# MIT-SPARK/Khronos

Hardware: AMD Instinct MI355X
Metric: active-window frames/sec (+ Mvoxel-updates/sec) at 1280x720 RGB-D+labels, 2 cm voxels (higher is better)
Workload: dtype f32

## Files before the change

### khronos_amd/csrc/khr_kernels_fusion.h

```cpp
#pragma once
#include "khr_device.h"

namespace khr {


constexpr int kTile = 16;
constexpr int kMaxTick = 8;

__device__ inline void ingestTile(const float* __restrict__ depth_in, const uint8_t* __restrict__ rgb_in,
                                  const int32_t* __restrict__ label_in, float* __restrict__ depth, float* __restrict__ range,
                                  uint32_t* __restrict__ rgba, int32_t* __restrict__ label, int32_t* __restrict__ dyn,
                                  float* __restrict__ tile_max, int tile, int tw, int W, int H, float fx, float fy, float cx,
                                  float cy, int range_mode, float* d_out, float* r_out) {
  const int tx = tile % tw, ty = tile / tw;
  const int u = tx * kTile + (threadIdx.x & 15), v = ty * kTile + (threadIdx.x >> 4);
  float r = 0.f, d = 0.f;
  if (u < W && v < H) {
    const int i = v * W + u;
    d = depth_in[i];
    if (d > 0.f && isfinite(d)) {
      if (range_mode == 0) {
        r = d;
      } else {
        const float x = (static_cast<float>(u) - cx) / fx, y = (static_cast<float>(v) - cy) / fy;
// ... 208 lines not shown
struct TickFrusta {
  float R[kMaxTick][9], t[kMaxTick][3], max_range[kMaxTick];
  DevFrustum fr[kMaxTick];
};
constexpr int kTickAllocThreads = 1024;
__global__ __launch_bounds__(kTickAllocThreads) void k_tick_alloc(DevMap m, DevParams p, TickFrusta tf, int ncam, int3 lo, int3 dim,
                                                   uint32_t* __restrict__ work, uint32_t list_stride,
                                                   uint32_t* __restrict__ new_list, uint32_t* __restrict__ tick_counts, int epoch) {
  const int total = dim.x * dim.y * dim.z;
  const int i = blockIdx.x * blockDim.x + threadIdx.x;
  uint32_t seen = 0u;
  int bx = 0, by = 0, bz = 0;
  if (i < total) {
    bx = lo.x + i % dim.x;
    by = lo.y + (i / dim.x) % dim.y;
    bz = lo.z + i / (dim.x * dim.y);
    if (ownerOf(bx, by, bz, p.world) == p.rank) {
      for (int k = 0; k < ncam; ++k) {
        const DevFrustum& fr = tf.fr[k];
        if (abs(bx - fr.bc.x) > fr.n_steps || abs(by - fr.bc.y) > fr.n_steps || abs(bz - fr.bc.z) > fr.n_steps) continue;
        const bool in = blockIsCandidate(p, fr, tf.R[k], tf.t[k], tf.max_range[k], bx, by, bz);
        if (in) seen |= 1u << k;
      }
    }
  }
  const bool visible = seen != 0u;
  uint32_t slot = kInvalidSlot;
  const uint64_t key = packKey(bx, by, bz);
  if (visible) slot = htLookup(m, key);
  const bool need = visible && slot == kInvalidSlot;
  const uint32_t fidx = waveAggInc(&m.counters[C_FREE_HEAD], need);
  bool got = false;
  if (need) {
    if (fidx < m.counters[C_N_FREE]) {
      slot = m.free_slots[fidx];
      got = true;
      m.blk_index[slot] = make_int4(bx, by, bz, epoch);
      m.blk_flags[slot] = BLK_LIVE | BLK_TRACK_DIRTY | BLK_ANY_KEEP;
      m.mesh_desc[slot] = MeshDesc{0u, 0u};
      htInsertUnique(m, key, slot);
      atomicMax(&m.counters[C_MAX_SLOT], slot + 1);
    } else {
      atomicAdd(&m.counters[C_POOL_EXHAUSTED], 1u);
      slot = kInvalidSlot;
    }
  }
  const uint32_t nidx = waveAggInc(&m.counters[C_N_NEW], got);
  if (got) new_list[nidx] = slot;
  if (slot == kInvalidSlot) seen = 0u;
  __shared__ uint32_t s_cnt[kMaxTick], s_base[kMaxTick];
  if (threadIdx.x < kMaxTick) s_cnt[threadIdx.x] = 0u;
  __syncthreads();
  uint32_t loff[kMaxTick];
#pragma unroll
  for (int k = 0; k < kMaxTick; ++k) {
    loff[k] = 0u;
    if (k < ncam) loff[k] = waveAggInc(&s_cnt[k], ((seen >> k) & 1u) != 0u);
  }
  __syncthreads();
  if (threadIdx.x < static_cast<uint32_t>(ncam)) {
    const uint32_t n = s_cnt[threadIdx.x];
    s_base[threadIdx.x] = n ? atomicAdd(&tick_counts[2 * threadIdx.x], n) : 0u;
  }
  if (threadIdx.x == 64) {
    uint32_t tot = 0u;
    for (int k = 0; k < ncam; ++k) tot += s_cnt[k];
    if (tot) atomicAdd(&m.counters[C_N_VISIBLE], tot);
  }
  __syncthreads();
#pragma unroll
  for (int k = 0; k < kMaxTick; ++k)
    if (k < ncam && ((seen >> k) & 1u)) work[static_cast<size_t>(k) * list_stride + s_base[k] + loff[k]] = slot;
}

__global__ void k_begin_integrate(DevMap m, int nvox, uint32_t* wg_stats) {
  if (blockIdx.x == 0) beginIntegrate(m, nvox, wg_stats);
}
__global__ void k_tick_begin(DevMap m, int nvox, uint32_t* wg_stats, uint32_t* tick_counts, uint32_t extra_calls) {
  beginIntegrate(m, nvox, wg_stats);
  if (threadIdx.x < 6 * kMaxTick) tick_counts[threadIdx.x] = 0u;
  if (threadIdx.x == 0) m.stats[S_CUM_CALLS] += extra_calls;
}

__device__ inline void cullBlocks(const DevMap& m, const DevParams& p, const DevFrame& f, const uint32_t* __restrict__ work,
                                  const uint32_t* __restrict__ n_work, FuseList out, uint32_t wpb,
                                  uint32_t* __restrict__ n_tsdf, const float* __restrict__ tile_max, int tw, int th,
                                  uint32_t bid, uint32_t nblk, uint32_t* __restrict__ item_mask = nullptr, uint32_t cam = 0u) {
  constexpr int kPerWg = 8;
  __shared__ uint4 s_blk[kPerWg];
  __shared__ uint16_t s_item[4][kPerWg * kBandSlots];
  __shared__ uint32_t s_nkeep, s_ccnt[4], s_off[4];
  const uint32_t n = *n_work;
  const uint32_t lane = threadIdx.x & 63;
  for (uint32_t base = bid * kPerWg; base < n; base += nblk * kPerWg) {
  if (threadIdx.x == 0) s_nkeep = 0;
  if (threadIdx.x < 4) s_ccnt[threadIdx.x] = 0;
  __syncthreads();
  for (uint32_t wi = base + (threadIdx.x >> 6); wi < min(n, base + kPerWg); wi += 4) {
    const uint32_t slot = work[wi];
    const int4 bi = m.blk_index[slot];
    bool keep = true;
    if (tile_max) {
      const float margin = 1e-3f;
      const float lo[3] = {static_cast<float>(bi.x) * p.bs + 0.5f * p.vs, static_cast<float>(bi.y) * p.bs + 0.5f * p.vs,
                           static_cast<float>(bi.z) * p.bs + 0.5f * p.vs};
      const float ext = p.bs - p.vs;
      float zmin = 1e30f, zmax = -1e30f, umin = 1e30f, umax = -1e30f, vmin = 1e30f, vmax = -1e30f;
      float pcs[8][3];
#pragma unroll
      for (int k = 0; k < 8; ++k) {
        xform(f.R, f.t, lo[0] + ((k & 1) ? ext : 0.f), lo[1] + ((k & 2) ? ext : 0.f), lo[2] + ((k & 4) ? ext : 0.f), pcs[k]);
        zmin = fminf(zmin, pcs[k][2]);
        zmax = fmaxf(zmax, pcs[k][2]);
      }
      if (zmax <= -margin) keep = false;
      if (zmin > f.max_range + margin) keep = false;
      if (p.range_mode == 0 && zmax < f.min_range - margin) keep = false;
      if (keep && zmin > 0.05f) {
#pragma unroll
        for (int k = 0; k < 8; ++k) {
          const float u = (pcs[k][0] * f.fx) / pcs[k][2] + f.cx, v = (pcs[k][1] * f.fy) / pcs[k][2] + f.cy;
          umin = fminf(umin, u); umax = fmaxf(umax, u);
          vmin = fminf(vmin, v); vmax = fmaxf(vmax, v);
        }
        if (umax < -1.f || vmax < -1.f || umin > static_cast<float>(f.W) || vmin > static_cast<float>(f.H)) {
          keep = false;
        } else {
          const int tx0 = max(0, (static_cast<int>(floorf(umin)) - 1) / kTile);
          const int ty0 = max(0, (static_cast<int>(floorf(vmin)) - 1) / kTile);
          const int tx1 = min(tw - 1, (static_cast<int>(ceilf(umax)) + 2) / kTile);
          const int ty1 = min(th - 1, (static_cast<int>(ceilf(vmax)) + 2) / kTile);
          if (tx1 >= tx0 && ty1 >= ty0) {
            const int nx = tx1 - tx0 + 1, nt = nx * (ty1 - ty0 + 1);
            float mr = 0.f;
            for (int t = lane; t < nt; t += 64) mr = fmaxf(mr, tile_max[(ty0 + t / nx) * tw + tx0 + t % nx]);
#pragma unroll
            for (int o = 32; o > 0; o >>= 1) mr = fmaxf(mr, __shfl_xor(mr, o));
            if (mr < zmin - p.trunc - margin) keep = false;
          }
        }
      }
    }
    if (keep) {
      uint32_t kslot = 0;
      if (lane == 0) {
        kslot = atomicAdd(&s_nkeep, 1u);
        s_blk[kslot] = make_uint4(slot, static_cast<uint32_t>(bi.x), static_cast<uint32_t>(bi.y), static_cast<uint32_t>(bi.z));
      }
      kslot = __shfl(kslot, 0);
      const uint32_t lpi = 64u / wpb, item = lane / lpi, sub = lane % lpi;
      bool ikeep = true;
      if (tile_max && (p.dbg & 256) == 0) {
        const float margin = 1e-3f;
        const int patches = (p.vps * p.vps) >> 6, rows = 64 / p.vps, zr = p.vps / (static_cast<int>(wpb) / patches);
        const int y0 = (static_cast<int>(item) % patches) * rows, z0 = (static_cast<int>(item) / patches) * zr;
        const float lo[3] = {static_cast<float>(bi.x) * p.bs + 0.5f * p.vs, static_cast<float>(bi.y) * p.bs + (static_cast<float>(y0) + 0.5f) * p.vs,
                             static_cast<float>(bi.z) * p.bs + (static_cast<float>(z0) + 0.5f) * p.vs};
        const float ex[3] = {p.bs - p.vs, static_cast<float>(rows - 1) * p.vs, static_cast<float>(zr - 1) * p.vs};
        float zmin = 1e30f, zmax = -1e30f, umin = 1e30f, umax = -1e30f, vmin = 1e30f, vmax = -1e30f;
        float pcs[8][3];
#pragma unroll
        for (int k = 0; k < 8; ++k) {
          xform(f.R, f.t, lo[0] + ((k & 1) ? ex[0] : 0.f), lo[1] + ((k & 2) ? ex[1] : 0.f), lo[2] + ((k & 4) ? ex[2] : 0.f), pcs[k]);
          zmin = fminf(zmin, pcs[k][2]);
          zmax = fmaxf(zmax, pcs[k][2]);
        }
        if (zmax <= -margin) ikeep = false;
        if (zmin > f.max_range + margin) ikeep = false;
        if (p.range_mode == 0 && zmax < f.min_range - margin) ikeep = false;
        if (ikeep && zmin > 0.05f) {
#pragma unroll
          for (int k = 0; k < 8; ++k) {
            const float iz = __builtin_amdgcn_rcpf(pcs[k][2]);
            const float u = (pcs[k][0] * f.fx) * iz + f.cx, v = (pcs[k][1] * f.fy) * iz + f.cy;
            umin = fminf(umin, u); umax = fmaxf(umax, u);
            vmin = fminf(vmin, v); vmax = fmaxf(vmax, v);
          }
          if (umax < -2.f || vmax < -2.f || umin > static_cast<float>(f.W) + 1.f || vmin > static_cast<float>(f.H) + 1.f) {
            ikeep = false;
          } else {
            const int tx0 = max(0, (static_cast<int>(floorf(umin)) - 2) / kTile);
            const int ty0 = max(0, (static_cast<int>(floorf(vmin)) - 2) / kTile);
            const int tx1 = min(tw - 1, (static_cast<int>(ceilf(umax)) + 3) / kTile);
            const int ty1 = min(th - 1, (static_cast<int>(ceilf(vmax)) + 3) / kTile);
            const int nx = tx1 - tx0 + 1, nt = nx * (ty1 - ty0 + 1);
            if (tx1 >= tx0 && ty1 >= ty0 && nt <= 16 * static_cast<int>(lpi)) {
              float m0 = 0.f, m1 = 0.f;
              int t = static_cast<int>(sub);
              for (; t + static_cast<int>(lpi) < nt; t += 2 * static_cast<int>(lpi)) {
                const int t2 = t + static_cast<int>(lpi);
                const float a = tile_max[(ty0 + t / nx) * tw + tx0 + t % nx];
                const float b = tile_max[(ty0 + t2 / nx) * tw + tx0 + t2 % nx];
                m0 = fmaxf(m0, a);
                m1 = fmaxf(m1, b);
              }
              if (t < nt) m0 = fmaxf(m0, tile_max[(ty0 + t / nx) * tw + tx0 + t % nx]);
              float mr = fmaxf(m0, m1);
              for (uint32_t o = 1; o < lpi; o <<= 1) mr = fmaxf(mr, __shfl_xor(mr, static_cast<int>(o)));
              if (mr < zmin - p.trunc - margin) ikeep = false;
            }
          }
        }
      }
      if (ikeep && sub == 0 && item_mask) {
        const size_t mi = static_cast<size_t>(slot) * wpb + item;
        const uint32_t sh = 8u * static_cast<uint32_t>(mi & 3);
        const uint32_t old = atomicOr(&item_mask[mi >> 2], (1u << cam) << sh);
        if ((old >> sh) & 0xffu) ikeep = false;
      }
      if (ikeep && sub == 0) {
        const uint32_t cls = fuseClass(m.blk_band[static_cast<size_t>(slot) * kBandSlots + item] & kItemBandMask);
        s_item[cls][atomicAdd(&s_ccnt[cls], 1u)] = static_cast<uint16_t>((kslot << 8) | item);
      }
    }
  }
  __syncthreads();
  if (threadIdx.x < 4) s_off[threadIdx.x] = s_ccnt[threadIdx.x] ? atomicAdd(&out.counts[threadIdx.x], s_ccnt[threadIdx.x]) : 0u;
  if (threadIdx.x == 0 && s_nkeep) atomicAdd(n_tsdf, s_nkeep);
  __syncthreads();
#pragma unroll
  for (uint32_t cls = 0; cls < 4; ++cls) {
    for (uint32_t i = threadIdx.x; i < s_ccnt[cls]; i += blockDim.x) {
      const uint32_t it = s_item[cls][i];
      uint4 d = s_blk[it >> 8];
      d.x |= (it & 0xffu) << 24;
      *fuseDescPtr(out, cls, s_off[cls] + i) = d;
    }
  }
  __syncthreads();
  }
}

__global__ __launch_bounds__(256) void k_cull_blocks(DevMap m, DevParams p, DevFrame f,
                                                    const uint32_t* __restrict__ work, FuseList out, uint32_t wpb,
                                                    const float* __restrict__ tile_max, int tw, int th) {
  cullBlocks(m, p, f, work, &m.counters[C_N_VISIBLE], out, wpb, &m.counters[C_N_TSDF], tile_max, tw, th, blockIdx.x, gridDim.x);
}

struct TickFrames {
  DevFrame f[kMaxTick];
  const float* tile_max[kMaxTick];
};
__global__ __launch_bounds__(256) void k_tick_cull(DevMap m, DevParams p, TickFrames t, const uint32_t* __restrict__ work,
                                                  uint32_t list_stride, uint4* __restrict__ desc, uint32_t desc_stride, uint32_t wpb,
                                                  uint32_t* __restrict__ tick_counts, int use_tiles, int tw, int th,
                                                  uint32_t* __restrict__ item_mask) {
  const int cam = blockIdx.y;
  const int lc = item_mask ? 0 : cam;
  FuseList out{desc + static_cast<size_t>(2 * lc) * desc_stride, desc + static_cast<size_t>(2 * lc + 1) * desc_stride, desc_stride,
               &tick_counts[2 * kMaxTick + 4 * lc]};
  cullBlocks(m, p, t.f[cam], work + static_cast<size_t>(cam) * list_stride, &tick_counts[2 * cam], out, wpb, &tick_counts[2 * cam + 1],
             use_tiles ? t.tile_max[cam] : nullptr, tw, th, blockIdx.x, gridDim.x, item_mask, static_cast<uint32_t>(cam));
}

__global__ __launch_bounds__(256) void k_alloc_list(DevMap m, const int* __restrict__ idx, int n,
                                                   uint32_t* __restrict__ new_list) {
  const int i = blockIdx.x * blockDim.x + threadIdx.x;
  bool need = false;
  int bx = 0, by = 0, bz = 0;
  if (i < n) {
    bx = idx[3 * i];
    by = idx[3 * i + 1];
    bz = idx[3 * i + 2];
    need = htLookup(m, packKey(bx, by, bz)) == kInvalidSlot;
  }
  const uint32_t fidx = waveAggInc(&m.counters[C_FREE_HEAD], need);
  bool got = false;
  uint32_t slot = kInvalidSlot;
  if (need) {
    if (fidx < m.counters[C_N_FREE]) {
      slot = m.free_slots[fidx];
      got = true;
      m.blk_index[slot] = make_int4(bx, by, bz, 0);
      m.blk_flags[slot] = BLK_LIVE | BLK_TRACK_DIRTY | BLK_ANY_KEEP;
      m.mesh_desc[slot] = MeshDesc{0u, 0u};
      htInsertUnique(m, packKey(bx, by, bz), slot);
      atomicMax(&m.counters[C_MAX_SLOT], slot + 1);
    } else {
      atomicAdd(&m.counters[C_POOL_EXHAUSTED], 1u);
    }
  }
  const uint32_t nidx = waveAggInc(&m.counters[C_N_NEW], got);
  if (got) new_list[nidx] = slot;
}

__global__ __launch_bounds__(256) void k_list_live(DevMap m, uint32_t* __restrict__ work, uint32_t* counter,
                                                  uint32_t require_flags, FuseList out = FuseList{nullptr, nullptr, 0u, nullptr},
                                                  uint32_t wpb = 0u) {
  const uint32_t s = blockIdx.x * blockDim.x + threadIdx.x;
  bool live = false;
  if (s < m.counters[C_MAX_SLOT]) {
    const uint32_t fl = m.blk_flags[s];
    live = (fl & BLK_LIVE) && ((fl & require_flags) == require_flags);
  }
  const uint32_t idx = waveAggInc(counter, live);
  if (live) work[idx] = s;
  if (out.a) {
    const unsigned long long mask = __ballot(live);
    if (mask) {
      const uint32_t lane = laneId();
      const int leader = __ffsll(static_cast<long long>(mask)) - 1;
      uint32_t base = 0;
      if (lane == static_cast<uint32_t>(leader)) base = atomicAdd(&out.counts[3], static_cast<uint32_t>(__popcll(mask)) * wpb);
      base = __shfl(base, leader) + static_cast<uint32_t>(__popcll(mask & ((1ull << lane) - 1ull))) * wpb;
      if (live) {
        const int4 bi = m.blk_index[s];
        for (uint32_t it = 0; it < wpb; ++it)
          *fuseDescPtr(out, 3u, base + it) =
              make_uint4(s | (it << 24), static_cast<uint32_t>(bi.x), static_cast<uint32_t>(bi.y), static_cast<uint32_t>(bi.z));
      }
    }
  }
}

__device__ inline void initBlocks(const DevMap& m, const DevParams& p, const uint32_t* __restrict__ new_list, uint32_t bid,
                                  uint32_t nblk) {
  const uint32_t n = m.counters[C_N_NEW];
  const int nv = p.nvox;
  for (uint32_t b = bid; b < n; b += nblk) {
    const size_t slot = new_list[b];
    const uint4 z = make_uint4(0, 0, 0, 0);
    uint4* d4 = reinterpret_cast<uint4*>(m.dist + slot * nv);
    uint4* w4 = reinterpret_cast<uint4*>(m.weight + slot * nv);
    uint4* c4 = reinterpret_cast<uint4*>(m.color + slot * nv);
    uint4* l4 = reinterpret_cast<uint4*>(m.sem_label + slot * nv);
    for (int i = threadIdx.x; i < nv / 4; i += blockDim.x) {
      d4[i] = z;
      w4[i] = z;
      c4[i] = z;
      if (p.with_semantics) l4[i] = z;
    }
    uint4* f4 = reinterpret_cast<uint4*>(m.vflags + slot * nv);
    for (int i = threadIdx.x; i < nv / 16; i += blockDim.x) f4[i] = z;
    if (threadIdx.x < kBandSlots) m.blk_band[slot * kBandSlots + threadIdx.x] = 0;
    if (p.with_tracking) {
      uint4* o4 = reinterpret_cast<uint4*>(m.last_obs + slot * nv);
      uint4* q4 = reinterpret_cast<uint4*>(m.last_occ + slot * nv);
      for (int i = threadIdx.x; i < nv / 2; i += blockDim.x) {
        o4[i] = z;
        q4[i] = z;
      }
      uint64_t* fb = m.freebits + slot * (nv / 64);
      for (int i = threadIdx.x; i < nv / 64; i += blockDim.x) {
        fb[i] = 0ull;
        m.obs[slot * (nv / 64) + i] = make_ulonglong2(0ull, 0ull);
      }
    }
  }
}

__global__ __launch_bounds__(256) void k_init_blocks(DevMap m, DevParams p, const uint32_t* __restrict__ new_list) {
  initBlocks(m, p, new_list, blockIdx.x, gridDim.x);
}

__global__ __launch_bounds__(256) void k_init_cull(DevMap m, DevParams p, DevFrame f, const uint32_t* __restrict__ new_list,
                                                  const uint32_t* __restrict__ work, FuseList out, uint32_t wpb,
                                                  const float* __restrict__ tile_max, int tw, int th, uint32_t n_cull) {
  if (blockIdx.x < n_cull)
    cullBlocks(m, p, f, work, &m.counters[C_N_VISIBLE], out, wpb, &m.counters[C_N_TSDF], tile_max, tw, th, blockIdx.x, n_cull);
  else
    initBlocks(m, p, new_list, blockIdx.x - n_cull, gridDim.x - n_cull);
}

__device__ inline uint32_t foldItemRecords(uint32_t* __restrict__ blk_flags, uint16_t* __restrict__ blk_band, uint32_t s) {
  static_assert(kBandSlots == 32, "record row = 4 x 16 bytes");
  uint4* const row = reinterpret_cast<uint4*>(blk_band + static_cast<size_t>(s) * kBandSlots);
  uint32_t any = 0u;
  uint4 r[4];
#pragma unroll
  for (int i = 0; i < 4; ++i) {
    r[i] = row[i];
    any |= r[i].x | r[i].y | r[i].z | r[i].w;
  }
  const uint32_t tm = static_cast<uint32_t>(kItemTouched) * 0x00010001u, nm = static_cast<uint32_t>(kItemNeg) * 0x00010001u;
  uint32_t fl = blk_flags[s];
  if ((any & tm) == 0u) return fl;
  fl |= BLK_UPDATED | BLK_MESH_UPDATED | BLK_TRACKING_UPDATED | ((any & nm) ? BLK_HAS_NEG : 0u);
  blk_flags[s] = fl;
  const uint32_t keep = static_cast<uint32_t>(kItemBandMask) * 0x00010001u;
#pragma unroll
  for (int i = 0; i < 4; ++i) row[i] = make_uint4(r[i].x & keep, r[i].y & keep, r[i].z & keep, r[i].w & keep);
  return fl;
}
__global__ __launch_bounds__(256) void k_tracking_select(DevMap m, uint64_t lim_active, uint64_t lim_free, int force_full,
                                                        uint32_t* __restrict__ proc, uint32_t* __restrict__ ef_list,
                                                        uint32_t* __restrict__ cnt ,
                                                        uint32_t* __restrict__ cnt_next, uint16_t* __restrict__ fold_band) {
  const uint32_t s = blockIdx.x * blockDim.x + threadIdx.x;
  if (s == 0) { cnt_next[0] = 0u; cnt_next[1] = 0u; }
  bool need = false, touched = false, reload = false;
  if (s < m.counters[C_MAX_SLOT]) {
    const uint32_t fl = fold_band ? foldItemRecords(m.blk_flags, fold_band, s) : m.blk_flags[s];
    if (fl & BLK_LIVE) {
      touched = fl & BLK_TRACKING_UPDATED;
      need = force_full || (fl & (BLK_TRACKING_UPDATED | BLK_TRACK_DIRTY));
      reload = need;
      if (!need) {
        const ulonglong2 lim = reinterpret_cast<const ulonglong2*>(m.trk_lim)[s];
        need = !(lim_active <= lim.x && lim_free <= lim.y);
      }
    }
  }
  const uint32_t ip = waveAggInc(&cnt[0], need);
  if (need) {
    proc[ip] = s | (reload ? 0x80000000u : 0u);
    reinterpret_cast<ulonglong2*>(m.trk_lim)[s] = make_ulonglong2(~0ull, ~0ull);
    m.blk_flags[s] = m.blk_flags[s] & ~(BLK_TRACKING_UPDATED | BLK_HAS_ACTIVE | BLK_TRACK_DIRTY | BLK_ANY_KEEP);
  }
  const uint32_t ie = waveAggInc(&cnt[1], touched);
  if (touched) ef_list[ie] = s;
}

template <int VPS, int CH>
__global__ __launch_bounds__(256) void k_tracking_update(DevMap m, DevParams p, uint64_t stamp, uint64_t prev_stamp,
                                                        uint64_t lim_active, uint64_t lim_free,
                                                        const uint32_t* __restrict__ proc, const uint32_t* __restrict__ n_proc) {
  constexpr int NV = VPS * VPS * VPS;
  __shared__ uint64_t s_min[2][4];
  __shared__ uint32_t s_bits;
  const uint32_t n = *n_proc * CH;
  for (uint32_t wi = blockIdx.x; wi < n; wi += gridDim.x) {
    const uint32_t pe = proc[wi / CH];
    const uint32_t s = pe & 0x7fffffffu;
    const bool reload = (pe >> 31) != 0u;
    const int g0 = static_cast<int>(wi % CH) * (NV / 4 / CH);
    const size_t slot = s;
    const float4* __restrict__ dist4 = reinterpret_cast<const float4*>(m.dist + slot * NV);
    const ulonglong2* __restrict__ lobs2 = reinterpret_cast<const ulonglong2*>(m.last_obs + slot * NV);
    uint64_t* __restrict__ locc = m.last_occ + slot * NV;
    uint32_t* __restrict__ vfl4 = reinterpret_cast<uint32_t*>(m.vflags + slot * NV);
    uint64_t* __restrict__ fb = m.freebits + slot * (NV / 64);
    bool any_active = false, any_keep = false;
    uint64_t a_min = ~0ull, f_min = ~0ull;
    if (threadIdx.x == 0) s_bits = 0u;
    constexpr int G = NV / 4 / CH / 256 > 0 ? NV / 4 / CH / 256 : 1;
    constexpr int GEND = NV / 4 / CH;
    float4 d_[G];
    ulonglong2 oa_[G], ob_[G], ca_[G], cb_[G], ow_[G];
    uint32_t v4_[G];
    uint32_t need_[G];
#pragma unroll
    for (int q = 0; q < G; ++q) {
      const int gl = threadIdx.x + 256 * q, g = g0 + gl;
      if (gl < GEND) {
// ... 268 lines not shown
```

### khronos_amd/csrc/khronos_amd.hip

```cpp
#include <hip/hip_runtime.h>
#include <hip/hip_ext.h>
#include <hipcub/hipcub.hpp>

#include <algorithm>
#include <array>
#include <atomic>
#include <chrono>
#include <memory>
#include <mutex>
#include <cmath>
#include <cstdarg>
#include <cstdio>
#include <climits>
#include <cstring>
#include <cstdlib>
#include <functional>
#include <map>
#include <string>
#include <thread>
#include <tuple>
#include <unordered_map>
#include <vector>

#include "../../include/khronos_amd.h"
// ... 1335 lines not shown
  if (!fc) return fail(KHR_EINVAL, "null frame copy");
  HIP_TRY(hipSetDevice(fc->device));
  HIP_TRY(hipEventSynchronize(fc->ready));
  const size_t n = fc->n;
  if (depth) HIP_TRY(hipMemcpy(depth, fc->f.depth, n * 4, hipMemcpyDeviceToHost));
  if (range) HIP_TRY(hipMemcpy(range, fc->f.range, n * 4, hipMemcpyDeviceToHost));
  if (labels) HIP_TRY(hipMemcpy(labels, fc->f.label, n * 4, hipMemcpyDeviceToHost));
  if (color_rgb || vertex_map) {
    DevTemp tmp;
    HIP_TRY(hipMalloc(&tmp.p, n * 12));
    if (color_rgb) {
      hipLaunchKernelGGL(k_rgba_to_rgb, dim3(static_cast<unsigned>((n + 255) / 256)), dim3(256), 0, nullptr, fc->f.rgba, tmp.as<uint8_t>(), static_cast<uint32_t>(n));
      HIP_TRY(hipMemcpy(color_rgb, tmp.p, n * 3, hipMemcpyDeviceToHost));
    }
    if (vertex_map) {
      hipLaunchKernelGGL(k_vertex_map, dim3(static_cast<unsigned>((n + 255) / 256)), dim3(256), 0, nullptr, fc->f, tmp.as<float>());
      HIP_TRY(hipMemcpy(vertex_map, tmp.p, n * 12, hipMemcpyDeviceToHost));
    }
  }
  return KHR_OK;
}

void khr_frame_copy_release(khr_frame_copy* fc) {
  if (!fc) return;
  hipSetDevice(fc->device);
  if (fc->ready) {
    hipEventSynchronize(fc->ready);
    hipEventDestroy(fc->ready);
  }
  bool pooled = false;
  {
    std::lock_guard<std::mutex> lock(fc->pool->mu);
    if (!fc->pool->dead && fc->pool->free.size() < 8) {
      fc->pool->free.emplace_back(fc->block, fc->bytes);
      pooled = true;
    }
  }
  if (!pooled) hipFree(fc->block);
  delete fc;
}

int khr_copy_frame_image(khr_ctx* c, int slot, int which, void* device_dst) {
  if (!c || !device_dst || slot < 0 || slot >= static_cast<int>(c->slots.size()) || !c->slots[slot].valid) return fail(KHR_EINVAL, "bad argument");
  if (which != 0 && which != 1) return fail(KHR_EINVAL, "which must be 0 (dynamic) or 1 (object)");
  HIP_TRY(hipSetDevice(c->device));
  FrameSlot& s = c->slots[slot];
  const size_t n = static_cast<size_t>(s.sensor.width) * s.sensor.height;
  if (which == 1 && !s.has_obj) {
    HIP_TRY(hipMemsetAsync(device_dst, 0, n * sizeof(int32_t), c->stream));
    return KHR_OK;
  }
  if (which == 1) {
    HIP_TRY(hipEventRecord(c->ev_aux_done, c->aux_stream));
    HIP_TRY(hipStreamWaitEvent(c->stream, c->ev_aux_done, 0));
  }
  HIP_TRY(hipMemcpyAsync(device_dst, which == 0 ? s.dyn : s.obj, n * sizeof(int32_t), hipMemcpyDeviceToDevice, c->stream));
  return KHR_OK;
}

int khr_download_frame_image(khr_ctx* c, int slot, int which, int32_t* image) {
  if (!c || !image || slot < 0 || slot >= static_cast<int>(c->slots.size()) || !c->slots[slot].valid) return fail(KHR_EINVAL, "bad argument");
  if (which != 0 && which != 1) return fail(KHR_EINVAL, "which must be 0 (dynamic) or 1 (object)");
  FrameSlot& s = c->slots[slot];
  const size_t n = static_cast<size_t>(s.sensor.width) * s.sensor.height;
  if (which == 1 && !s.has_obj) {
    std::memset(image, 0, n * sizeof(int32_t));
    return KHR_OK;
  }
  if (which == 1) HIP_TRY(hipStreamSynchronize(c->aux_stream));
  HIP_TRY(hipMemcpyAsync(image, which == 0 ? s.dyn : s.obj, n * sizeof(int32_t), hipMemcpyDeviceToHost, c->stream));
  HIP_TRY(hipStreamSynchronize(c->stream));
  return KHR_OK;
}

static int integrateAlloc(khr_ctx* c, FrameSlot& s, const DevFrame& f, int allocate_blocks) {
  DevMap& m = c->m;
  if (!c->begun) hipLaunchKernelGGL(k_begin_integrate, dim3(1), dim3(256), 0, c->stream, m, c->p.nvox, c->d_wg_stats);
  c->begun = false;
  if (allocate_blocks) {
    ScopedTimer tm(c, 3);
    const DevFrustum fr = makeFrustum(c, f);
    const int S = 2 * fr.n_steps + 1;
    const size_t total = static_cast<size_t>(S) * S * S;
    hipLaunchKernelGGL(k_alloc_visible, dim3(gridFor(total)), dim3(256), 0, c->stream, m, c->p, f, fr, c->d_work, c->d_new,
                       c->d_pinned + 2, c->seed_publish_pending ? c->seed_ticket : 0u, &m.counters[C_N_VISIBLE], 0);
    c->seed_publish_pending = false;
    hipLaunchKernelGGL(k_init_cull, dim3(1024 + 1024), dim3(256), 0, c->stream, m, c->p, f, c->d_new, c->d_work,
                       FuseList{c->d_work4, c->d_work4 + c->item_cap, c->item_cap, &m.counters[C_N_ITEMS0]}, c->wpb,
                       c->cfg.disable_culling ? nullptr : s.vTileMax(), s.tw, s.th, 1024u);
    c->host_index_valid = false, ++c->map_gen;
  } else {
    hipLaunchKernelGGL(k_list_live, dim3(gridFor(m.capacity)), dim3(256), 0, c->stream, m, c->d_work,
                       &m.counters[C_N_VISIBLE], 0u, FuseList{c->d_work4, c->d_work4 + c->item_cap, c->item_cap, &m.counters[C_N_ITEMS0]},
                       c->wpb);
  }
  HIP_TRY(hipGetLastError());
  return KHR_OK;
}

struct UpdateLists {
  FuseList list{nullptr, nullptr, 0u, nullptr};
};

static int fuseGrid(khr_ctx* c, const void* kernel, int group, int block) {
  static std::map<std::pair<int, const void*>, int> cache;
  static std::mutex cache_mu;
  std::lock_guard<std::mutex> lock(cache_mu);
  const std::pair<int, const void*> key{c->device, kernel};
  auto it = cache.find(key);
  if (it != cache.end()) return it->second;
  int per_cu = 0, cus = 256;
  if (hipOccupancyMaxActiveBlocksPerMultiprocessor(&per_cu, kernel, block, 0) != hipSuccess || per_cu < 1) per_cu = 1;
  per_cu = std::min(per_cu, std::max(1, kUpdateWavesPerCu / (block / 64)));
  hipDeviceProp_t prop;
  if (hipGetDeviceProperties(&prop, c->device) == hipSuccess && prop.multiProcessorCount > 0) cus = prop.multiProcessorCount;
  per_cu = std::min(per_cu, 8);
  int grid = std::min(kUpdateStatSlots, per_cu * cus);
  grid = std::max(8 * group, grid / (8 * group) * (8 * group));
  cache[key] = grid;
  return grid;
}

static int fuse2Grid(khr_ctx* c, const void* kern, int wpw) {
  static std::map<std::pair<int, const void*>, int> cache;
  static std::mutex mu;
  std::lock_guard<std::mutex> lock(mu);
  const std::pair<int, const void*> key{c->device, kern};
  auto it = cache.find(key);
  if (it != cache.end()) return it->second;
  int per_cu = 0;
  if (hipOccupancyMaxActiveBlocksPerMultiprocessor(&per_cu, kern, 64 * wpw, 0) != hipSuccess || per_cu < 1) per_cu = 1;
  hipDeviceProp_t prop;
  int cus = 256;
  if (hipGetDeviceProperties(&prop, c->device) == hipSuccess && prop.multiProcessorCount > 0) cus = prop.multiProcessorCount;
  const int grid = std::min(kUpdateStatSlots, per_cu * cus) / 8 * 8;
  cache[key] = grid;
  return grid;
}

static void fillFuseFrame(const khr_ctx* c, const FrameSlot& s, const DevFrame& f, int use_mask, int object_id, FuseFrame* a) {
  a->range = f.range; a->dyn = f.dyn; a->rgba = f.rgba; a->label = f.label; a->obj = f.obj;
  a->W = f.W; a->H = f.H; a->fx = f.fx; a->fy = f.fy; a->cx = f.cx; a->cy = f.cy; a->min_range = f.min_range; a->max_range = f.max_range;
  std::memcpy(a->R, f.R, sizeof(a->R));
  std::memcpy(a->t, f.t, sizeof(a->t));
  a->stamp = f.stamp;
  a->use_mask = (use_mask && !s.dyn_clean) ? 1 : 0;
  a->has_color = f.has_color;
  a->object_id = object_id;
  a->do_sem = (c->p.with_semantics && ((c->p.sem_mode == 1) ? (object_id >= 0 && f.obj != nullptr) : (f.has_label != 0))) ? 1 : 0;
  a->tile_max = s.vTileMax();
  a->tw = s.tw;
  a->th = s.th;
}
static void fillFuseMap(khr_ctx* c, FuseArgs* a) {
  DevMap& m = c->m;
  a->blk_index = m.blk_index; a->blk_flags = m.blk_flags; a->dist = m.dist; a->weight = m.weight; a->last_obs = m.last_obs; a->obs = m.obs;
  a->color = m.color; a->vflags = m.vflags; a->sem_label = m.sem_label; a->lik = m.lik; a->wg_stats = c->d_wg_stats;
  a->blk_band = m.blk_band;
  a->vs = c->p.vs; a->bs = c->p.bs; a->trunc = c->p.trunc; a->dropoff_eps = c->p.dropoff_eps; a->max_weight = c->p.max_weight;
  a->adaptive_diff = c->p.adaptive_diff; a->log_match = c->p.log_match; a->log_nomatch = c->p.log_nomatch;
  a->interp = c->p.interp; a->range_mode = c->p.range_mode; a->use_dropoff = c->p.use_dropoff; a->const_weight = c->p.const_weight;
  a->with_tracking = c->p.with_tracking;
  a->K = c->p.K; a->KS = c->p.KS; a->sem_mode = c->p.sem_mode;
  a->band_mode = c->cfg.max_frame_pixels <= 640u * 480u ? 0 : 1;
  a->sink = c->d_fuse_sink;
  a->blend_pre = c->cfg.color_blend_weight != 0;
}

static int integrateUpdateMulti(khr_ctx* c, khr_ctx* src, const int* src_slots, const int* object_ids, int n_frames, int use_mask) {
  if (c->cfg.voxels_per_side != 8 || n_frames < 2 || n_frames > kMaxMultiFrames) return 1;
  FuseArgs a{};
  fillFuseMap(c, &a);
// ... 4384 lines not shown
```

Measured before the change: 4020.

## Fuse block allocation, new-block init and frustum culling into one kernel

Replaces the separate k_alloc_visible and k_init_cull launches with a single k_alloc_cull kernel. In it, one wave per workgroup tests 64 candidate blocks, allocates and zero-initialises new ones, then all 16 waves run the block and item culling tests, staging results in shared memory before appending them to the global lists with batched atomics. This removes one launch, the global round-trip of the visible and new lists, and the grid-wide dependency between the two stages. In exchange, many 1024-thread workgroups have idle lanes when few candidates are visible, and zeroing new blocks is serialised inside each workgroup.

```diff
diff --git a/khronos_amd/csrc/khr_kernels_fusion.h b/khronos_amd/csrc/khr_kernels_fusion.h
--- a/khronos_amd/csrc/khr_kernels_fusion.h
+++ b/khronos_amd/csrc/khr_kernels_fusion.h
@@ -314,6 +314,112 @@
   if (threadIdx.x == 0) m.stats[S_CUM_CALLS] += extra_calls;
 }
 
+__device__ inline bool cullBlockKeep(const DevParams& p, const DevFrame& f, const int4 bi, const float* __restrict__ tile_max, int tw,
+                                     int th, uint32_t lane) {
+  bool keep = true;
+  if (tile_max) {
+    const float margin = 1e-3f;
+    const float lo[3] = {static_cast<float>(bi.x) * p.bs + 0.5f * p.vs, static_cast<float>(bi.y) * p.bs + 0.5f * p.vs,
+                         static_cast<float>(bi.z) * p.bs + 0.5f * p.vs};
+    const float ext = p.bs - p.vs;
+    float zmin = 1e30f, zmax = -1e30f, umin = 1e30f, umax = -1e30f, vmin = 1e30f, vmax = -1e30f;
+    float pcs[8][3];
+#pragma unroll
+    for (int k = 0; k < 8; ++k) {
+      xform(f.R, f.t, lo[0] + ((k & 1) ? ext : 0.f), lo[1] + ((k & 2) ? ext : 0.f), lo[2] + ((k & 4) ? ext : 0.f), pcs[k]);
+      zmin = fminf(zmin, pcs[k][2]);
+      zmax = fmaxf(zmax, pcs[k][2]);
+    }
+    if (zmax <= -margin) keep = false;
+    if (zmin > f.max_range + margin) keep = false;
+    if (p.range_mode == 0 && zmax < f.min_range - margin) keep = false;
+    if (keep && zmin > 0.05f) {
+#pragma unroll
+      for (int k = 0; k < 8; ++k) {
+        const float u = (pcs[k][0] * f.fx) / pcs[k][2] + f.cx, v = (pcs[k][1] * f.fy) / pcs[k][2] + f.cy;
+        umin = fminf(umin, u); umax = fmaxf(umax, u);
+        vmin = fminf(vmin, v); vmax = fmaxf(vmax, v);
+      }
+      if (umax < -1.f || vmax < -1.f || umin > static_cast<float>(f.W) || vmin > static_cast<float>(f.H)) {
+        keep = false;
+      } else {
+        const int tx0 = max(0, (static_cast<int>(floorf(umin)) - 1) / kTile);
+        const int ty0 = max(0, (static_cast<int>(floorf(vmin)) - 1) / kTile);
+        const int tx1 = min(tw - 1, (static_cast<int>(ceilf(umax)) + 2) / kTile);
+        const int ty1 = min(th - 1, (static_cast<int>(ceilf(vmax)) + 2) / kTile);
+        if (tx1 >= tx0 && ty1 >= ty0) {
+          const int nx = tx1 - tx0 + 1, nt = nx * (ty1 - ty0 + 1);
+          float mr = 0.f;
+          for (int t = lane; t < nt; t += 64) mr = fmaxf(mr, tile_max[(ty0 + t / nx) * tw + tx0 + t % nx]);
+#pragma unroll
+          for (int o = 32; o > 0; o >>= 1) mr = fmaxf(mr, __shfl_xor(mr, o));
+          if (mr < zmin - p.trunc - margin) keep = false;
+        }
+      }
+    }
+  }
+  return keep;
+}
+
+__device__ inline bool cullItemKeep(const DevParams& p, const DevFrame& f, const int4 bi, uint32_t wpb, const float* __restrict__ tile_max,
+                                    int tw, int th, uint32_t lane) {
+  const uint32_t lpi = 64u / wpb, item = lane / lpi, sub = lane % lpi;
+  bool ikeep = true;
+  if (tile_max && (p.dbg & 256) == 0) {
+    const float margin = 1e-3f;
+    const int patches = (p.vps * p.vps) >> 6, rows = 64 / p.vps, zr = p.vps / (static_cast<int>(wpb) / patches);
+    const int y0 = (static_cast<int>(item) % patches) * rows, z0 = (static_cast<int>(item) / patches) * zr;
+    const float lo[3] = {static_cast<float>(bi.x) * p.bs + 0.5f * p.vs, static_cast<float>(bi.y) * p.bs + (static_cast<float>(y0) + 0.5f) * p.vs,
+                         static_cast<float>(bi.z) * p.bs + (static_cast<float>(z0) + 0.5f) * p.vs};
+    const float ex[3] = {p.bs - p.vs, static_cast<float>(rows - 1) * p.vs, static_cast<float>(zr - 1) * p.vs};
+    float zmin = 1e30f, zmax = -1e30f, umin = 1e30f, umax = -1e30f, vmin = 1e30f, vmax = -1e30f;
+    float pcs[8][3];
+#pragma unroll
+    for (int k = 0; k < 8; ++k) {
+      xform(f.R, f.t, lo[0] + ((k & 1) ? ex[0] : 0.f), lo[1] + ((k & 2) ? ex[1] : 0.f), lo[2] + ((k & 4) ? ex[2] : 0.f), pcs[k]);
+      zmin = fminf(zmin, pcs[k][2]);
+      zmax = fmaxf(zmax, pcs[k][2]);
+    }
+    if (zmax <= -margin) ikeep = false;
+    if (zmin > f.max_range + margin) ikeep = false;
+    if (p.range_mode == 0 && zmax < f.min_range - margin) ikeep = false;
+    if (ikeep && zmin > 0.05f) {
+#pragma unroll
+      for (int k = 0; k < 8; ++k) {
+        const float iz = __builtin_amdgcn_rcpf(pcs[k][2]);
+        const float u = (pcs[k][0] * f.fx) * iz + f.cx, v = (pcs[k][1] * f.fy) * iz + f.cy;
+        umin = fminf(umin, u); umax = fmaxf(umax, u);
+        vmin = fminf(vmin, v); vmax = fmaxf(vmax, v);
+      }
+      if (umax < -2.f || vmax < -2.f || umin > static_cast<float>(f.W) + 1.f || vmin > static_cast<float>(f.H) + 1.f) {
+        ikeep = false;
+      } else {
+        const int tx0 = max(0, (static_cast<int>(floorf(umin)) - 2) / kTile);
+        const int ty0 = max(0, (static_cast<int>(floorf(vmin)) - 2) / kTile);
+        const int tx1 = min(tw - 1, (static_cast<int>(ceilf(umax)) + 3) / kTile);
+        const int ty1 = min(th - 1, (static_cast<int>(ceilf(vmax)) + 3) / kTile);
+        const int nx = tx1 - tx0 + 1, nt = nx * (ty1 - ty0 + 1);
+        if (tx1 >= tx0 && ty1 >= ty0 && nt <= 16 * static_cast<int>(lpi)) {
+          float m0 = 0.f, m1 = 0.f;
+          int t = static_cast<int>(sub);
+          for (; t + static_cast<int>(lpi) < nt; t += 2 * static_cast<int>(lpi)) {
+            const int t2 = t + static_cast<int>(lpi);
+            const float a = tile_max[(ty0 + t / nx) * tw + tx0 + t % nx];
+            const float b = tile_max[(ty0 + t2 / nx) * tw + tx0 + t2 % nx];
+            m0 = fmaxf(m0, a);
+            m1 = fmaxf(m1, b);
+          }
+          if (t < nt) m0 = fmaxf(m0, tile_max[(ty0 + t / nx) * tw + tx0 + t % nx]);
+          float mr = fmaxf(m0, m1);
+          for (uint32_t o = 1; o < lpi; o <<= 1) mr = fmaxf(mr, __shfl_xor(mr, static_cast<int>(o)));
+          if (mr < zmin - p.trunc - margin) ikeep = false;
+        }
+      }
+    }
+  }
+  return ikeep;
+}
+
 __device__ inline void cullBlocks(const DevMap& m, const DevParams& p, const DevFrame& f, const uint32_t* __restrict__ work,
                                   const uint32_t* __restrict__ n_work, FuseList out, uint32_t wpb,
                                   uint32_t* __restrict__ n_tsdf, const float* __restrict__ tile_max, int tw, int th,
@@ -331,49 +437,7 @@
   for (uint32_t wi = base + (threadIdx.x >> 6); wi < min(n, base + kPerWg); wi += 4) {
     const uint32_t slot = work[wi];
     const int4 bi = m.blk_index[slot];
-    bool keep = true;
-    if (tile_max) {
-      const float margin = 1e-3f;
-      const float lo[3] = {static_cast<float>(bi.x) * p.bs + 0.5f * p.vs, static_cast<float>(bi.y) * p.bs + 0.5f * p.vs,
-                           static_cast<float>(bi.z) * p.bs + 0.5f * p.vs};
-      const float ext = p.bs - p.vs;
-      float zmin = 1e30f, zmax = -1e30f, umin = 1e30f, umax = -1e30f, vmin = 1e30f, vmax = -1e30f;
-      float pcs[8][3];
-#pragma unroll
-      for (int k = 0; k < 8; ++k) {
-        xform(f.R, f.t, lo[0] + ((k & 1) ? ext : 0.f), lo[1] + ((k & 2) ? ext : 0.f), lo[2] + ((k & 4) ? ext : 0.f), pcs[k]);
-        zmin = fminf(zmin, pcs[k][2]);
-        zmax = fmaxf(zmax, pcs[k][2]);
-      }
-      if (zmax <= -margin) keep = false;
-      if (zmin > f.max_range + margin) keep = false;
-      if (p.range_mode == 0 && zmax < f.min_range - margin) keep = false;
-      if (keep && zmin > 0.05f) {
-#pragma unroll
-        for (int k = 0; k < 8; ++k) {
-          const float u = (pcs[k][0] * f.fx) / pcs[k][2] + f.cx, v = (pcs[k][1] * f.fy) / pcs[k][2] + f.cy;
-          umin = fminf(umin, u); umax = fmaxf(umax, u);
-          vmin = fminf(vmin, v); vmax = fmaxf(vmax, v);
-        }
-        if (umax < -1.f || vmax < -1.f || umin > static_cast<float>(f.W) || vmin > static_cast<float>(f.H)) {
-          keep = false;
-        } else {
-          const int tx0 = max(0, (static_cast<int>(floorf(umin)) - 1) / kTile);
-          const int ty0 = max(0, (static_cast<int>(floorf(vmin)) - 1) / kTile);
-          const int tx1 = min(tw - 1, (static_cast<int>(ceilf(umax)) + 2) / kTile);
-          const int ty1 = min(th - 1, (static_cast<int>(ceilf(vmax)) + 2) / kTile);
-          if (tx1 >= tx0 && ty1 >= ty0) {
-            const int nx = tx1 - tx0 + 1, nt = nx * (ty1 - ty0 + 1);
-            float mr = 0.f;
-            for (int t = lane; t < nt; t += 64) mr = fmaxf(mr, tile_max[(ty0 + t / nx) * tw + tx0 + t % nx]);
-#pragma unroll
-            for (int o = 32; o > 0; o >>= 1) mr = fmaxf(mr, __shfl_xor(mr, o));
-            if (mr < zmin - p.trunc - margin) keep = false;
-          }
-        }
-      }
-    }
-    if (keep) {
+    if (cullBlockKeep(p, f, bi, tile_max, tw, th, lane)) {
       uint32_t kslot = 0;
       if (lane == 0) {
         kslot = atomicAdd(&s_nkeep, 1u);
@@ -381,59 +445,7 @@
       }
       kslot = __shfl(kslot, 0);
       const uint32_t lpi = 64u / wpb, item = lane / lpi, sub = lane % lpi;
-      bool ikeep = true;
-      if (tile_max && (p.dbg & 256) == 0) {
-        const float margin = 1e-3f;
-        const int patches = (p.vps * p.vps) >> 6, rows = 64 / p.vps, zr = p.vps / (static_cast<int>(wpb) / patches);
-        const int y0 = (static_cast<int>(item) % patches) * rows, z0 = (static_cast<int>(item) / patches) * zr;
-        const float lo[3] = {static_cast<float>(bi.x) * p.bs + 0.5f * p.vs, static_cast<float>(bi.y) * p.bs + (static_cast<float>(y0) + 0.5f) * p.vs,
-                             static_cast<float>(bi.z) * p.bs + (static_cast<float>(z0) + 0.5f) * p.vs};
-        const float ex[3] = {p.bs - p.vs, static_cast<float>(rows - 1) * p.vs, static_cast<float>(zr - 1) * p.vs};
-        float zmin = 1e30f, zmax = -1e30f, umin = 1e30f, umax = -1e30f, vmin = 1e30f, vmax = -1e30f;
-        float pcs[8][3];
-#pragma unroll
-        for (int k = 0; k < 8; ++k) {
-          xform(f.R, f.t, lo[0] + ((k & 1) ? ex[0] : 0.f), lo[1] + ((k & 2) ? ex[1] : 0.f), lo[2] + ((k & 4) ? ex[2] : 0.f), pcs[k]);
-          zmin = fminf(zmin, pcs[k][2]);
-          zmax = fmaxf(zmax, pcs[k][2]);
-        }
-        if (zmax <= -margin) ikeep = false;
-        if (zmin > f.max_range + margin) ikeep = false;
-        if (p.range_mode == 0 && zmax < f.min_range - margin) ikeep = false;
-        if (ikeep && zmin > 0.05f) {
-#pragma unroll
-          for (int k = 0; k < 8; ++k) {
-            const float iz = __builtin_amdgcn_rcpf(pcs[k][2]);
-            const float u = (pcs[k][0] * f.fx) * iz + f.cx, v = (pcs[k][1] * f.fy) * iz + f.cy;
-            umin = fminf(umin, u); umax = fmaxf(umax, u);
-            vmin = fminf(vmin, v); vmax = fmaxf(vmax, v);
-          }
-          if (umax < -2.f || vmax < -2.f || umin > static_cast<float>(f.W) + 1.f || vmin > static_cast<float>(f.H) + 1.f) {
-            ikeep = false;
-          } else {
-            const int tx0 = max(0, (static_cast<int>(floorf(umin)) - 2) / kTile);
-            const int ty0 = max(0, (static_cast<int>(floorf(vmin)) - 2) / kTile);
-            const int tx1 = min(tw - 1, (static_cast<int>(ceilf(umax)) + 3) / kTile);
-            const int ty1 = min(th - 1, (static_cast<int>(ceilf(vmax)) + 3) / kTile);
-            const int nx = tx1 - tx0 + 1, nt = nx * (ty1 - ty0 + 1);
-            if (tx1 >= tx0 && ty1 >= ty0 && nt <= 16 * static_cast<int>(lpi)) {
-              float m0 = 0.f, m1 = 0.f;
-              int t = static_cast<int>(sub);
-              for (; t + static_cast<int>(lpi) < nt; t += 2 * static_cast<int>(lpi)) {
-                const int t2 = t + static_cast<int>(lpi);
-                const float a = tile_max[(ty0 + t / nx) * tw + tx0 + t % nx];
-                const float b = tile_max[(ty0 + t2 / nx) * tw + tx0 + t2 % nx];
-                m0 = fmaxf(m0, a);
-                m1 = fmaxf(m1, b);
-              }
-              if (t < nt) m0 = fmaxf(m0, tile_max[(ty0 + t / nx) * tw + tx0 + t % nx]);
-              float mr = fmaxf(m0, m1);
-              for (uint32_t o = 1; o < lpi; o <<= 1) mr = fmaxf(mr, __shfl_xor(mr, static_cast<int>(o)));
-              if (mr < zmin - p.trunc - margin) ikeep = false;
-            }
-          }
-        }
-      }
+      bool ikeep = cullItemKeep(p, f, bi, wpb, tile_max, tw, th, lane);
       if (ikeep && sub == 0 && item_mask) {
         const size_t mi = static_cast<size_t>(slot) * wpb + item;
         const uint32_t sh = 8u * static_cast<uint32_t>(mi & 3);
@@ -545,53 +557,153 @@
   }
 }
 
+__device__ inline void initBlock(const DevMap& m, const DevParams& p, size_t slot) {
+  const int nv = p.nvox;
+  const uint4 z = make_uint4(0, 0, 0, 0);
+  uint4* d4 = reinterpret_cast<uint4*>(m.dist + slot * nv);
+  uint4* w4 = reinterpret_cast<uint4*>(m.weight + slot * nv);
+  uint4* c4 = reinterpret_cast<uint4*>(m.color + slot * nv);
+  uint4* l4 = reinterpret_cast<uint4*>(m.sem_label + slot * nv);
+  for (int i = threadIdx.x; i < nv / 4; i += blockDim.x) {
+    d4[i] = z;
+    w4[i] = z;
+    c4[i] = z;
+    if (p.with_semantics) l4[i] = z;
+  }
+  uint4* f4 = reinterpret_cast<uint4*>(m.vflags + slot * nv);
+  for (int i = threadIdx.x; i < nv / 16; i += blockDim.x) f4[i] = z;
+  if (threadIdx.x < kBandSlots) m.blk_band[slot * kBandSlots + threadIdx.x] = 0;
+  if (p.with_tracking) {
+    uint4* o4 = reinterpret_cast<uint4*>(m.last_obs + slot * nv);
+    uint4* q4 = reinterpret_cast<uint4*>(m.last_occ + slot * nv);
+    for (int i = threadIdx.x; i < nv / 2; i += blockDim.x) {
+      o4[i] = z;
+      q4[i] = z;
+    }
+    uint64_t* fb = m.freebits + slot * (nv / 64);
+    for (int i = threadIdx.x; i < nv / 64; i += blockDim.x) {
+      fb[i] = 0ull;
+      m.obs[slot * (nv / 64) + i] = make_ulonglong2(0ull, 0ull);
+    }
+  }
+}
 __device__ inline void initBlocks(const DevMap& m, const DevParams& p, const uint32_t* __restrict__ new_list, uint32_t bid,
                                   uint32_t nblk) {
   const uint32_t n = m.counters[C_N_NEW];
-  const int nv = p.nvox;
-  for (uint32_t b = bid; b < n; b += nblk) {
-    const size_t slot = new_list[b];
-    const uint4 z = make_uint4(0, 0, 0, 0);
-    uint4* d4 = reinterpret_cast<uint4*>(m.dist + slot * nv);
-    uint4* w4 = reinterpret_cast<uint4*>(m.weight + slot * nv);
-    uint4* c4 = reinterpret_cast<uint4*>(m.color + slot * nv);
-    uint4* l4 = reinterpret_cast<uint4*>(m.sem_label + slot * nv);
-    for (int i = threadIdx.x; i < nv / 4; i += blockDim.x) {
-      d4[i] = z;
-      w4[i] = z;
-      c4[i] = z;
-      if (p.with_semantics) l4[i] = z;
-    }
-    uint4* f4 = reinterpret_cast<uint4*>(m.vflags + slot * nv);
-    for (int i = threadIdx.x; i < nv / 16; i += blockDim.x) f4[i] = z;
-    if (threadIdx.x < kBandSlots) m.blk_band[slot * kBandSlots + threadIdx.x] = 0;
-    if (p.with_tracking) {
-      uint4* o4 = reinterpret_cast<uint4*>(m.last_obs + slot * nv);
-      uint4* q4 = reinterpret_cast<uint4*>(m.last_occ + slot * nv);
-      for (int i = threadIdx.x; i < nv / 2; i += blockDim.x) {
-        o4[i] = z;
-        q4[i] = z;
-      }
-      uint64_t* fb = m.freebits + slot * (nv / 64);
-      for (int i = threadIdx.x; i < nv / 64; i += blockDim.x) {
-        fb[i] = 0ull;
-        m.obs[slot * (nv / 64) + i] = make_ulonglong2(0ull, 0ull);
-      }
-    }
-  }
+  for (uint32_t b = bid; b < n; b += nblk) initBlock(m, p, new_list[b]);
 }
 
 __global__ __launch_bounds__(256) void k_init_blocks(DevMap m, DevParams p, const uint32_t* __restrict__ new_list) {
   initBlocks(m, p, new_list, blockIdx.x, gridDim.x);
 }
 
-__global__ __launch_bounds__(256) void k_init_cull(DevMap m, DevParams p, DevFrame f, const uint32_t* __restrict__ new_list,
-                                                  const uint32_t* __restrict__ work, FuseList out, uint32_t wpb,
-                                                  const float* __restrict__ tile_max, int tw, int th, uint32_t n_cull) {
-  if (blockIdx.x < n_cull)
-    cullBlocks(m, p, f, work, &m.counters[C_N_VISIBLE], out, wpb, &m.counters[C_N_TSDF], tile_max, tw, th, blockIdx.x, n_cull);
-  else
-    initBlocks(m, p, new_list, blockIdx.x - n_cull, gridDim.x - n_cull);
+constexpr int kAllocCands = 64;
+constexpr int kAllocThreads = 1024;
+__global__ __launch_bounds__(kAllocThreads) void k_alloc_cull(DevMap m, DevParams p, DevFrame f, DevFrustum fr,
+                                                             uint32_t* __restrict__ work, uint32_t* __restrict__ new_list,
+                                                             volatile uint32_t* host_seed, uint32_t seed_ticket, FuseList out,
+                                                             uint32_t wpb, const float* __restrict__ tile_max, int tw, int th) {
+  static_assert(kAllocCands == 64, "the allocating lanes are one wave");
+  __shared__ uint4 s_cand[kAllocCands];
+  __shared__ uint32_t s_new[kAllocCands];
+  __shared__ uint16_t s_ent[kAllocCands * kBandSlots];
+  __shared__ uint32_t s_nvis, s_nnew, s_nkeep, s_ccnt[4], s_off[4], s_wbase, s_nbase;
+  if (seed_ticket && blockIdx.x == 0 && threadIdx.x == 0) publishSeedCount(m, host_seed, seed_ticket);
+  if (threadIdx.x == 64) s_nkeep = 0u;
+  if (threadIdx.x >= 64 && threadIdx.x < 68) s_ccnt[threadIdx.x - 64] = 0u;
+  const uint32_t lane = threadIdx.x & 63, wave = threadIdx.x >> 6;
+  if (wave == 0) {
+    const int S = 2 * fr.n_steps + 1;
+    const int total = S * S * S;
+    const int i = blockIdx.x * kAllocCands + static_cast<int>(lane);
+    bool visible = false;
+    int bx = 0, by = 0, bz = 0;
+    if (i < total) {
+      const int dx = i % S - fr.n_steps, dy = (i / S) % S - fr.n_steps, dz = i / (S * S) - fr.n_steps;
+      bx = fr.bc.x + dx;
+      by = fr.bc.y + dy;
+      bz = fr.bc.z + dz;
+      const bool in = blockIsCandidate(p, fr, f.R, f.t, f.max_range, bx, by, bz);
+      visible = in && ownerOf(bx, by, bz, p.world) == p.rank;
+    }
+    uint32_t slot = kInvalidSlot;
+    const uint64_t key = packKey(bx, by, bz);
+    if (visible) slot = htLookup(m, key);
+    const bool need = visible && slot == kInvalidSlot;
+    const uint32_t fidx = waveAggInc(&m.counters[C_FREE_HEAD], need);
+    bool got = false;
+    if (need) {
+      if (fidx < m.counters[C_N_FREE]) {
+        slot = m.free_slots[fidx];
+        got = true;
+        m.blk_index[slot] = make_int4(bx, by, bz, 0);
+        m.blk_flags[slot] = BLK_LIVE | BLK_TRACK_DIRTY | BLK_ANY_KEEP;
+        m.mesh_desc[slot] = MeshDesc{0u, 0u};
+        htInsertUnique(m, key, slot);
+        atomicMax(&m.counters[C_MAX_SLOT], slot + 1);
+      } else {
+        atomicAdd(&m.counters[C_POOL_EXHAUSTED], 1u);
+        slot = kInvalidSlot;
+      }
+    }
+    const unsigned long long got_mask = __ballot(got);
+    if (got) s_new[__popcll(got_mask & ((1ull << lane) - 1ull))] = slot;
+    const bool emit = visible && slot != kInvalidSlot;
+    const unsigned long long emit_mask = __ballot(emit);
+    if (emit)
+      s_cand[__popcll(emit_mask & ((1ull << lane) - 1ull))] =
+          make_uint4(slot, static_cast<uint32_t>(bx), static_cast<uint32_t>(by), static_cast<uint32_t>(bz));
+    if (lane == 0) {
+      s_nvis = static_cast<uint32_t>(__popcll(emit_mask));
+      s_nnew = static_cast<uint32_t>(__popcll(got_mask));
+    }
+  }
+  __syncthreads();
+  const uint32_t n_vis = s_nvis, n_new = s_nnew;
+  if (n_vis == 0u) return;
+  if (n_new) {
+    for (uint32_t b = 0; b < n_new; ++b) initBlock(m, p, s_new[b]);
+    __syncthreads();
+  }
+  for (uint32_t ci = wave; ci < n_vis; ci += kAllocThreads / 64) {
+    const uint4 cd = s_cand[ci];
+    const uint32_t slot = cd.x;
+    const int4 bi = make_int4(static_cast<int>(cd.y), static_cast<int>(cd.z), static_cast<int>(cd.w), 0);
+    uint16_t ent = 0xffffu;
+    const uint32_t lpi = 64u / wpb, item = lane / lpi, sub = lane % lpi;
+    const uint16_t band = m.blk_band[static_cast<size_t>(slot) * kBandSlots + item];
+    if (cullBlockKeep(p, f, bi, tile_max, tw, th, lane)) {
+      if (lane == 0) atomicAdd(&s_nkeep, 1u);
+      if (cullItemKeep(p, f, bi, wpb, tile_max, tw, th, lane) && sub == 0) {
+        const uint32_t cls = fuseClass(band & kItemBandMask);
+        ent = static_cast<uint16_t>((atomicAdd(&s_ccnt[cls], 1u) << 2) | cls);
+      }
+    }
+    if (sub == 0) s_ent[ci * wpb + item] = ent;
+  }
+  __syncthreads();
+  static_assert(C_N_ITEMS0 % 2 == 0, "the class counts are added in 8-byte pairs");
+  if ((threadIdx.x == 0 || threadIdx.x == 64)) {
+    const uint32_t c0 = threadIdx.x == 0 ? 0u : 2u;
+    const unsigned long long add = static_cast<unsigned long long>(s_ccnt[c0]) | (static_cast<unsigned long long>(s_ccnt[c0 + 1]) << 32);
+    const unsigned long long old = add ? atomicAdd(reinterpret_cast<unsigned long long*>(out.counts + c0), add) : 0ull;
+    s_off[c0] = static_cast<uint32_t>(old);
+    s_off[c0 + 1] = static_cast<uint32_t>(old >> 32);
+  }
+  if (threadIdx.x == 128) s_wbase = atomicAdd(&m.counters[C_N_VISIBLE], n_vis);
+  if (threadIdx.x == 192) s_nbase = n_new ? atomicAdd(&m.counters[C_N_NEW], n_new) : 0u;
+  if (threadIdx.x == 256 && s_nkeep) atomicAdd(&m.counters[C_N_TSDF], s_nkeep);
+  __syncthreads();
+  if (threadIdx.x < n_vis) work[s_wbase + threadIdx.x] = s_cand[threadIdx.x].x;
+  if (threadIdx.x >= 64 && threadIdx.x - 64 < n_new) new_list[s_nbase + threadIdx.x - 64] = s_new[threadIdx.x - 64];
+  for (uint32_t e = threadIdx.x; e < n_vis * wpb; e += kAllocThreads) {
+    const uint32_t ent = s_ent[e];
+    if (ent == 0xffffu) continue;
+    const uint32_t cls = ent & 3u;
+    uint4 d = s_cand[e / wpb];
+    d.x |= (e % wpb) << 24;
+    *fuseDescPtr(out, cls, s_off[cls] + (ent >> 2)) = d;
+  }
 }
 
 __device__ inline uint32_t foldItemRecords(uint32_t* __restrict__ blk_flags, uint16_t* __restrict__ blk_band, uint32_t s) {
diff --git a/khronos_amd/csrc/khronos_amd.hip b/khronos_amd/csrc/khronos_amd.hip
--- a/khronos_amd/csrc/khronos_amd.hip
+++ b/khronos_amd/csrc/khronos_amd.hip
@@ -1441,12 +1441,11 @@
     const DevFrustum fr = makeFrustum(c, f);
     const int S = 2 * fr.n_steps + 1;
     const size_t total = static_cast<size_t>(S) * S * S;
-    hipLaunchKernelGGL(k_alloc_visible, dim3(gridFor(total)), dim3(256), 0, c->stream, m, c->p, f, fr, c->d_work, c->d_new,
-                       c->d_pinned + 2, c->seed_publish_pending ? c->seed_ticket : 0u, &m.counters[C_N_VISIBLE], 0);
+    hipLaunchKernelGGL(k_alloc_cull, dim3(static_cast<unsigned>((total + kAllocCands - 1) / kAllocCands)), dim3(kAllocThreads), 0, c->stream, m,
+                       c->p, f, fr, c->d_work, c->d_new, c->d_pinned + 2, c->seed_publish_pending ? c->seed_ticket : 0u,
+                       FuseList{c->d_work4, c->d_work4 + c->item_cap, c->item_cap, &m.counters[C_N_ITEMS0]}, c->wpb,
+                       c->cfg.disable_culling ? nullptr : s.vTileMax(), s.tw, s.th);
     c->seed_publish_pending = false;
-    hipLaunchKernelGGL(k_init_cull, dim3(1024 + 1024), dim3(256), 0, c->stream, m, c->p, f, c->d_new, c->d_work,
-                       FuseList{c->d_work4, c->d_work4 + c->item_cap, c->item_cap, &m.counters[C_N_ITEMS0]}, c->wpb,
-                       c->cfg.disable_culling ? nullptr : s.vTileMax(), s.tw, s.th, 1024u);
     c->host_index_valid = false, ++c->map_gen;
   } else {
     hipLaunchKernelGGL(k_list_live, dim3(gridFor(m.capacity)), dim3(256), 0, c->stream, m, c->d_work,
```

Result: slower. 3911 (-2.7%).
